# VITA-Group/Open-L2O

Measured on NVIDIA H100. Metric: coordinate-updates/sec (N_params x unroll_steps), higher is better.
Workload: dtype f32

## Files before the change

open_l2o_b200/csrc/cwlstm_tc.cuh:

```cuda
#pragma once
#include "cwlstm_common.cuh"
#include "l2o_internal.h"

namespace l2o {
namespace tc {

constexpr int kH = 20;
constexpr int kN = 4 * kH;
constexpr int kTile = 64;
constexpr int kU = 5;
constexpr int kFwdWG = 3;
constexpr int kFwdThreads = 128 * kFwdWG;
template <int N>
struct IC {
  static constexpr int value = N;
};

template <class C>
struct Geo {
  static constexpr bool FC = C::FC;
  static constexpr int ColH1 = FC ? 24 : 4, ColH2 = FC ? 44 : 24;
  static constexpr int ColOne = FC ? 20 : C::F;
  static constexpr int KB = FC ? 8 : 6;
  static constexpr int L1Lo = 0, L1Hi = FC ? 6 : 3;
  static constexpr int L2Lo = FC ? 2 : 0, L2Hi = KB;
  static constexpr int K1 = 8 * (L1Hi - L1Lo), K2 = 8 * (L2Hi - L2Lo);
  static constexpr int N1 = FC ? 48 : 24, N2 = 48;
  static constexpr int B1Floats = K1 * kN, B2Floats = K2 * kN, T1Floats = kN * N1, T2Floats = kN * N2;
  static constexpr int FwdFloats = 2 * (B1Floats + B2Floats);
  static constexpr int AllFloats = FwdFloats + 2 * (T1Floats + T2Floats);
  static_assert(!FC || C::F == 20, "fc preprocessing: dim 20");
  static_assert(FC || C::F <= 3, "feature chunk: at most 3 features");
};
constexpr int kImgMaxFloats = Geo<Cfg<L2O_PRE_FC, 2, 20, 20, 20>>::AllFloats;

__device__ __forceinline__ uint32_t smem_u32(const void* p) { return (uint32_t)__cvta_generic_to_shared(p); }

__device__ __forceinline__ void mbar_init(uint64_t* bar, uint32_t count) {
  asm volatile("mbarrier.init.shared::cta.b64 [%0], %1;" ::"r"(smem_u32(bar)), "r"(count));
}
__device__ __forceinline__ void mbar_expect_tx(uint64_t* bar, uint32_t bytes) {
  asm volatile("mbarrier.arrive.expect_tx.shared::cta.b64 _, [%0], %1;" ::"r"(smem_u32(bar)), "r"(bytes) : "memory");
}
__device__ __forceinline__ void mbar_wait(uint64_t* bar, uint32_t parity) {
  asm volatile(
      "{\n\t"
      ".reg .pred p;\n\t"
      "WAIT_LOOP:\n\t"
      "mbarrier.try_wait.parity.shared::cta.b64 p, [%0], %1;\n\t"
      "@p bra WAIT_DONE;\n\t"
      "bra WAIT_LOOP;\n\t"
      "WAIT_DONE:\n\t"
      "}\n" ::"r"(smem_u32(bar)),
      "r"(parity)
      : "memory");
}
__device__ __forceinline__ void fence_barrier_init() { asm volatile("fence.mbarrier_init.release.cluster;" ::: "memory"); }
__device__ __forceinline__ void fence_proxy_async() { asm volatile("fence.proxy.async.shared::cta;" ::: "memory"); }
__device__ __forceinline__ void tma_bulk_g2s(void* dst, const void* src, uint32_t bytes, uint64_t* bar) {
  asm volatile("cp.async.bulk.shared::cluster.global.mbarrier::complete_tx::bytes [%0], [%1], %2, [%3];" ::"r"(
                   smem_u32(dst)),
               "l"(src), "r"(bytes), "r"(smem_u32(bar))
               : "memory");
}
__device__ __forceinline__ void stage_image(float* dst, const float* src, uint32_t bytes, uint64_t* bar) {
  if (threadIdx.x == 0) {
    mbar_expect_tx(bar, bytes);
    tma_bulk_g2s(dst, src, bytes, bar);
  }
  mbar_wait(bar, 0);
}

__device__ __forceinline__ void wg_fence() { asm volatile("wgmma.fence.sync.aligned;" ::: "memory"); }
__device__ __forceinline__ void wg_commit() { asm volatile("wgmma.commit_group.sync.aligned;" ::: "memory"); }
template <int N>
__device__ __forceinline__ void wg_wait() {
  asm volatile("wgmma.wait_group.sync.aligned %0;" ::"n"(N) : "memory");
}

__device__ __forceinline__ uint64_t make_desc(uint32_t saddr, uint32_t lbo, uint32_t sbo) {
  return (uint64_t)((saddr & 0x3FFFFu) >> 4) | ((uint64_t)(lbo >> 4) << 16) | ((uint64_t)(sbo >> 4) << 32);
}
__device__ __forceinline__ uint64_t img_desc(const float* p, int ncols) {
  return make_desc(smem_u32(p), (uint32_t)(ncols / 8) * 128u, 128u);
}
__host__ __device__ constexpr uint64_t img_kstep(int ncols) { return (uint64_t)((2 * (ncols / 8) * 128) >> 4); }

#define L2O_ACC8(b) "+f"(d[b]), "+f"(d[b + 1]), "+f"(d[b + 2]), "+f"(d[b + 3]), "+f"(d[b + 4]), "+f"(d[b + 5]), \
                    "+f"(d[b + 6]), "+f"(d[b + 7])
__device__ __forceinline__ void mma_rs_n80(float* d, const uint32_t* a, uint64_t b, uint32_t acc) {
  asm volatile(
      "{\n\t.reg .pred p;\n\tsetp.ne.b32 p, %45, 0;\n\t"
      "wgmma.mma_async.sync.aligned.m64n80k8.f32.tf32.tf32 "
      "{%0,%1,%2,%3,%4,%5,%6,%7,%8,%9,%10,%11,%12,%13,%14,%15,%16,%17,%18,%19,"
      "%20,%21,%22,%23,%24,%25,%26,%27,%28,%29,%30,%31,%32,%33,%34,%35,%36,%37,%38,%39}, "
      "{%40,%41,%42,%43}, %44, p, 1, 1;\n\t}\n"
      : L2O_ACC8(0), L2O_ACC8(8), L2O_ACC8(16), L2O_ACC8(24), L2O_ACC8(32)
      : "r"(a[0]), "r"(a[1]), "r"(a[2]), "r"(a[3]), "l"(b), "r"(acc));
}
__device__ __forceinline__ void mma_rs_n48(float* d, const uint32_t* a, uint64_t b, uint32_t acc) {
  asm volatile(
      "{\n\t.reg .pred p;\n\tsetp.ne.b32 p, %29, 0;\n\t"
      "wgmma.mma_async.sync.aligned.m64n48k8.f32.tf32.tf32 "
      "{%0,%1,%2,%3,%4,%5,%6,%7,%8,%9,%10,%11,%12,%13,%14,%15,%16,%17,%18,%19,%20,%21,%22,%23}, "
      "{%24,%25,%26,%27}, %28, p, 1, 1;\n\t}\n"
      : L2O_ACC8(0), L2O_ACC8(8), L2O_ACC8(16)
      : "r"(a[0]), "r"(a[1]), "r"(a[2]), "r"(a[3]), "l"(b), "r"(acc));
}
__device__ __forceinline__ void mma_rs_n24(float* d, const uint32_t* a, uint64_t b, uint32_t acc) {
  asm volatile(
      "{\n\t.reg .pred p;\n\tsetp.ne.b32 p, %17, 0;\n\t"
      "wgmma.mma_async.sync.aligned.m64n24k8.f32.tf32.tf32 "
      "{%0,%1,%2,%3,%4,%5,%6,%7,%8,%9,%10,%11}, "
      "{%12,%13,%14,%15}, %16, p, 1, 1;\n\t}\n"
      : L2O_ACC8(0), "+f"(d[8]), "+f"(d[9]), "+f"(d[10]), "+f"(d[11])
      : "r"(a[0]), "r"(a[1]), "r"(a[2]), "r"(a[3]), "l"(b), "r"(acc));
}
template <int N>
__device__ __forceinline__ void mma_rs(float* d, const uint32_t* a, uint64_t b, uint32_t acc) {
  static_assert(N == 80 || N == 48 || N == 24, "wgmma width");
  if constexpr (N == 80) mma_rs_n80(d, a, b, acc);
  else if constexpr (N == 48) mma_rs_n48(d, a, b, acc);
  else mma_rs_n24(d, a, b, acc);
}

__device__ __forceinline__ float to_tf32(float x) {
  uint32_t r;
  asm("cvt.rna.tf32.f32 %0, %1;" : "=r"(r) : "f"(x));
  return __uint_as_float(r);
}
__device__ __forceinline__ void split_tf32(float x, uint32_t& hi, uint32_t& lo) {
  hi = __float_as_uint(x) & 0xFFFFE000u;
  lo = __float_as_uint(x - __uint_as_float(hi));
}

__host__ __device__ constexpr int vec_unit(int c, int base) { return 5 * ((c - base) & 3) + ((c - base) >> 2); }
__host__ __device__ constexpr int unit_col(int u, int base) { return base + 4 * (u % 5) + u / 5; }
__host__ __device__ constexpr int gate_ref_col(int n) {
  return (2 * ((n >> 3) & 1) + (n & 1)) * kH + 5 * ((n & 7) >> 1) + (n >> 4);
}
__host__ __device__ constexpr int dx_gate_col(int k) { return (k & ~7) + 2 * (k & 3) + ((k >> 2) & 1); }
__host__ __device__ constexpr int dx_group(int c) { return c / 24; }
__host__ __device__ constexpr int dx_unit(int c) {
  return 2 * ((c % 24) >> 3) + (c & 1) >= 5 ? -1 : 5 * ((c & 7) >> 1) + 2 * ((c % 24) >> 3) + (c & 1);
}
__host__ __device__ constexpr int img_index(int k, int n, int ncols) {
  return ((k >> 2) * (ncols / 8) + (n >> 3)) * 32 + (n & 7) * 4 + (k & 3);
}

template <class C>
__device__ __forceinline__ float ext_weight(const float* __restrict__ theta, bool l2, int c, int n) {
  using G = Geo<C>;
  const int col = gate_ref_col(n);
  if (c == G::ColOne) return theta[(l2 ? C::O_B2 : C::O_B1) + col];
  const bool in_h1 = c >= G::ColH1 && c < G::ColH1 + kH, in_h2 = c >= G::ColH2 && c < G::ColH2 + kH;
  if (!l2) {
    if (in_h1) return theta[C::O_W1 + (C::F + vec_unit(c, G::ColH1)) * C::G1 + col];
    if (G::FC && c < kH) return theta[C::O_W1 + vec_unit(c, 0) * C::G1 + col];
    if (!G::FC && c < C::F) return theta[C::O_W1 + c * C::G1 + col];
    return 0.f;
  }
  if (in_h1) return theta[C::O_W2 + vec_unit(c, G::ColH1) * C::G2 + col];
  if (in_h2) return theta[C::O_W2 + (kH + vec_unit(c, G::ColH2)) * C::G2 + col];
  return 0.f;
}
template <class C>
__host__ __device__ constexpr int dx_operand_col(bool l2, int c) {
  using G = Geo<C>;
  return l2 ? unit_col(dx_unit(c), dx_group(c) == 0 ? G::ColH1 : G::ColH2)
            : unit_col(dx_unit(c), dx_group(c) == 0 ? G::ColH1 : 0);
}

template <class C>
__global__ void prep_weights_kernel(const float* __restrict__ theta, float* __restrict__ img, int with_transposed) {
  static_assert(C::H1 == kH && C::H2 == kH && (C::F <= 3 || C::FC), "tc engine: LSTM-20x2, F <= 3 or fc(20)");
  using G = Geo<C>;
  const int nb = (G::K1 + G::K2) * kN;
  const int nt = with_transposed ? kN * (G::N1 + G::N2) : 0;
  for (int e = blockIdx.x * blockDim.x + threadIdx.x; e < nb + nt; e += gridDim.x * blockDim.x) {
    float w;
    float* hi;
    int off, idx;
    if (e < nb) {
      const bool l2 = e >= G::K1 * kN;
      const int ee = l2 ? e - G::K1 * kN : e;
      const int k = ee / kN, n = ee % kN;
      w = ext_weight<C>(theta, l2, 8 * (l2 ? G::L2Lo : G::L1Lo) + k, n);
      hi = img + (l2 ? 2 * G::B1Floats : 0);
      off = l2 ? G::B2Floats : G::B1Floats;
      idx = img_index(k, n, kN);
    } else {
      const int e2 = e - nb;
      const bool l2 = e2 >= kN * G::N1;
      const int nc = l2 ? G::N2 : G::N1;
      const int ee = l2 ? e2 - kN * G::N1 : e2;
      const int k = ee / nc, n = ee % nc;
      w = dx_unit(n) < 0 ? 0.f : ext_weight<C>(theta, l2, dx_operand_col<C>(l2, n), dx_gate_col(k));
      hi = img + G::FwdFloats + (l2 ? 2 * G::T1Floats : 0);
      off = l2 ? G::T2Floats : G::T1Floats;
      idx = img_index(k, n, nc);
    }
    const float h = to_tf32(w);
    hi[idx] = h;
    hi[off + idx] = to_tf32(w - h);
  }
}

template <int KB>
struct Frag {
  uint32_t hi[KB][4], lo[KB][4];
  __device__ __forceinline__ void zero() {
#pragma unroll
    for (int k = 0; k < KB; ++k)
#pragma unroll
      for (int r = 0; r < 4; ++r) { hi[k][r] = 0u; lo[k][r] = 0u; }
  }
  __device__ __forceinline__ void put_at(int c, int rh, float v) {
    split_tf32(v, hi[c / 8][((c / 4) & 1) * 2 + rh], lo[c / 8][((c / 4) & 1) * 2 + rh]);
  }
  __device__ __forceinline__ float get_at(int c, int rh) const {
    return __uint_as_float(hi[c / 8][((c / 4) & 1) * 2 + rh]) + __uint_as_float(lo[c / 8][((c / 4) & 1) * 2 + rh]);
  }
  template <int COL>
  __device__ __forceinline__ void put(int rh, float v) {
    static_assert(COL % 4 == 0 && COL / 8 < KB, "fragment column");
    put_at(COL, rh, v);
  }
  template <int BASE>
  __device__ __forceinline__ void put_vec(int rh, const float* v) {
    static_assert(BASE % 4 == 0 && (BASE + 19) / 8 < KB, "fragment column");
#pragma unroll
    for (int s = 0; s < kU; ++s) put_at(BASE + 4 * s, rh, v[s]);
  }
};

template <int N, int KB, int LO, int HI>
__device__ __forceinline__ void mma3(float* d, const Frag<KB>& f, uint64_t bh, uint64_t bl) {
  constexpr uint64_t step = img_kstep(N);
#pragma unroll
  for (int kb = LO; kb < HI; ++kb) {
    const uint64_t o = (uint64_t)(kb - LO) * step;
    mma_rs<N>(d, f.lo[kb], bh + o, kb > LO ? 1u : 0u);
    mma_rs<N>(d, f.hi[kb], bl + o, 1u);
    mma_rs<N>(d, f.hi[kb], bh + o, 1u);
  }
}

__host__ __device__ constexpr int acc_idx(int s, int g, int rh) { return 4 * (2 * s + (g >> 1)) + 2 * rh + (g & 1); }

constexpr float kLog2e = 1.4426950408889634f;
__device__ __forceinline__ void lstm_point_fwd(float zi, float zj, float zf, float zo, float& c, float& h) {
  const float Ei = ex2_approx(fminf(-kLog2e * zi, 40.f));
  const float Ej = ex2_approx(fminf(-2.f * kLog2e * zj, 40.f));
  const float Qf = 1.0f + ex2_approx(fminf(fmaf(-kLog2e, zf, -kLog2e), 40.f));
  const float Pij = (1.0f + Ei) * (1.0f + Ej);
  const float cn = fmaf(c, Pij, (1.0f - Ej) * Qf) * rcp_approx(Pij * Qf);
  c = cn;
  const float Ec = ex2_approx(fminf(-2.f * kLog2e * cn, 63.f));
  const float Eo = ex2_approx(fminf(-kLog2e * zo, 63.f));
  h = (1.0f - Ec) * rcp_approx((1.0f + Ec) * (1.0f + Eo));
}
__device__ __forceinline__ float elu_fast(float av) {
  const float em = ex2_approx(kLog2e * av) - 1.0f;
  const float ep = av * fmaf(av, fmaf(av, fmaf(av, 1.0f / 24.0f, 1.0f / 6.0f), 0.5f), 1.0f);
  return av > 0.f ? av : (av > -0.0625f ? ep : em);
}

__device__ __forceinline__ void load5(const float* __restrict__ p, int q, float* v) {
#pragma unroll
  for (int s = 0; s < kU; ++s) v[s] = p[5 * q + s];
}
__device__ __forceinline__ void store5(float* __restrict__ p, int q, const float* v) {
#pragma unroll
  for (int s = 0; s < kU; ++s) p[5 * q + s] = v[s];
}
__device__ __forceinline__ float quad_sum(float v) {
  v += __shfl_xor_sync(0xffffffffu, v, 1);
  return v + __shfl_xor_sync(0xffffffffu, v, 2);
}
__device__ __forceinline__ float from_row(float v, int lane, int rh) {
  return __shfl_sync(0xffffffffu, v, (lane & ~3) | rh);
}

struct FwdExtra {
  const int32_t* step_ptr;
  int32_t t_offset;
  float p_fixed;
};

template <class C>
struct SmemF {
  float img[Geo<C>::FwdFloats];
  float wo[kH + 4];
  float win[64];
  uint64_t wbar;
};
template <class C>
__host__ __device__ constexpr size_t adamc_offset() {
  return (sizeof(SmemF<C>) + 15) & ~(size_t)15;
}
template <class C>
__host__ __device__ constexpr size_t fwd_smem_bytes(int T) {
  return adamc_offset<C>() + (C::FC ? (size_t)T * 2 * sizeof(float) : 0);
}
__device__ __forceinline__ double warp_sum_pairs_d(double v) {
  v += __shfl_xor_sync(0xffffffffu, v, 16);
  v += __shfl_xor_sync(0xffffffffu, v, 8);
  v += __shfl_xor_sync(0xffffffffu, v, 4);
  return v + __shfl_xor_sync(0xffffffffu, v, 1);
}

template <class C, bool FAST = false, int OPT = L2O_OPT_NONE, bool CKPT = false>
__global__ void __launch_bounds__(kFwdThreads, 1) unroll_fwd_kernel(l2o_unroll_args a, NetRt rt, const float* __restrict__ img,
                                                                     float* __restrict__ state_out, FwdExtra ex) {
  static_assert(!FAST || (!C::FC && OPT != L2O_OPT_NONE), "the full-tile forward is the DM nets' with an optimizee");
  using G = Geo<C>;
  extern __shared__ __align__(128) unsigned char smem_raw[];
  SmemF<C>& S = *reinterpret_cast<SmemF<C>*>(smem_raw);
  const int T = a.T;
  const int64_t n = a.n;
  const bool in_kernel_opt = FAST || a.opt_kind != L2O_OPT_NONE;
  const int opt_kind = FAST ? OPT : a.opt_kind;
  const bool want_fx = in_kernel_opt && a.fx != nullptr;
  const bool adam_mode = C::NIN == 2 && a.m != nullptr;
  const bool has_ckpt = FAST ? CKPT : a.ckpt != nullptr;
  const bool has_grec = FAST ? CKPT : a.g_rec != nullptr;
  const bool tanh_out = !FAST && rt.tanh_output;
  const bool has_delta = !FAST && a.delta_seq != nullptr;
  const bool has_labels = !FAST && a.labels != nullptr;
  float* adamc = reinterpret_cast<float*>(smem_raw + adamc_offset<C>());

  if (threadIdx.x < kH) S.wo[threadIdx.x] = a.theta[C::O_WO + threadIdx.x];
  if (threadIdx.x == kH) S.wo[kH] = a.theta[C::O_BO];
  if constexpr (C::FC) {
    static_assert(!C::FC || C::NIN == 2, "fc nets here are RNNprop nets (two inputs)");
    if (threadIdx.x >= 32 && threadIdx.x < 92) S.win[threadIdx.x - 32] = a.theta[C::O_WIN + threadIdx.x - 32];
    if (adam_mode) {
      const int step0 = ex.step_ptr ? *ex.step_ptr + ex.t_offset : a.step0;
      for (int t = threadIdx.x; t < T; t += blockDim.x) {
        const float p = (ex.step_ptr == nullptr && ex.p_fixed > 0.f) ? ex.p_fixed : (float)(step0 + t);
        adamc[2 * t] = 1.0f - powf(a.beta1, p);
        adamc[2 * t + 1] = 1.0f - powf(a.beta2, p);
      }
    }
  }
  if (threadIdx.x == 0) {
    mbar_init(&S.wbar, 1);
    fence_barrier_init();
  }
  __syncthreads();
// ... 261 lines not shown
```

open_l2o_b200/csrc/cwlstm_tc_bwd.cuh:

```cuda
#pragma once
#include <type_traits>
#include "cwlstm_tc.cuh"

namespace l2o {
namespace tcb {

using namespace tc;

constexpr int kBwdWG = 2;
constexpr int kBwdThreads = 128 * kBwdWG;
constexpr uint32_t kXaLBO = 8 * 128;
constexpr uint32_t kXbLBO = 10 * 128;
constexpr uint32_t kXaBytes = 8 * kXaLBO;
constexpr uint32_t kXbBytes = 8 * kXbLBO;
constexpr int kBlkL1 = 5, kRowOne2 = 63;

__device__ __forceinline__ void split_bf16x2(float v0, float v1, uint32_t& hi, uint32_t& lo) {
  asm("cvt.rn.bf16x2.f32 %0, %1, %2;" : "=r"(hi) : "f"(v1), "f"(v0));
  const float r0 = v0 - __uint_as_float(hi << 16), r1 = v1 - __uint_as_float(hi & 0xFFFF0000u);
  asm("cvt.rn.bf16x2.f32 %0, %1, %2;" : "=r"(lo) : "f"(r1), "f"(r0));
}
__device__ __forceinline__ void stsm_x4_trans(uint32_t sa, uint32_t r0, uint32_t r1, uint32_t r2, uint32_t r3) {
  asm volatile("stmatrix.sync.aligned.m8n8.x4.trans.shared.b16 [%0], {%1, %2, %3, %4};" ::"r"(sa), "r"(r0), "r"(r1),
               "r"(r2), "r"(r3)
// ... 194 lines not shown
      split_bf16x2(z[4 * j + 2], z[4 * j + 3], h1, l1);
      stsm_x4_trans(lb + (uint32_t)j * 128, h0, h1, l0, l1);
    }
  };
  auto dx_dw = [&](auto ncols, float* z, float* x, uint64_t th, uint64_t tl, uint64_t xah, uint64_t xal) {
    constexpr int NX = decltype(ncols)::value;
    uint32_t fh[kN / 8][4], fl[kN / 8][4];
#pragma unroll
    for (int j = 0; j < kN / 8; ++j) {
      split_tf32(z[4 * j + 0], fh[j][0], fl[j][0]);
      split_tf32(z[4 * j + 2], fh[j][1], fl[j][1]);
      split_tf32(z[4 * j + 1], fh[j][2], fl[j][2]);
      split_tf32(z[4 * j + 3], fh[j][3], fl[j][3]);
    }
    constexpr uint64_t step = img_kstep(NX);
    wg_fence();
#pragma unroll
    for (int j = 0; j < kN / 8; ++j) {
      mma_rs<NX>(x, fl[j], th + j * step, j > 0 ? 1u : 0u);
      mma_rs<NX>(x, fh[j], tl + j * step, 1u);
      mma_rs<NX>(x, fh[j], th + j * step, 1u);
    }
    wg_commit();
    constexpr uint64_t sa = (2 * kXaLBO) >> 4, sb = (2 * kXbLBO) >> 4;
#pragma unroll
    for (int kk = 0; kk < tc::kTile / 16; ++kk) {
      mma_ss_bf16_n80(dw, xal + kk * sa, xbh + kk * sb);
      mma_ss_bf16_n80(dw, xah + kk * sa, xbl + kk * sb);
      mma_ss_bf16_n80(dw, xah + kk * sa, xbh + kk * sb);
    }
    wg_commit();
    wg_wait<1>();
  };
  auto flush_dw = [&]() {
    wg_wait<0>();
#pragma unroll
    for (int rh = 0; rh < 2; ++rh) {
      const int r = dw_row<C, MODE>(kx + 8 * rh);
#pragma unroll
      for (int j = 0; j < kN / 8; ++j)
#pragma unroll
        for (int e = 0; e < 2; ++e) {
          float& v = dw[4 * j + 2 * rh + e];
          if (r >= 0 && v != 0.f) atomicAdd(&a.dtheta[r + gate_ref_col(8 * j + 2 * q + e)], (double)v);
          v = 0.f;
        }
    }
  };

  for (int64_t tile = (int64_t)blockIdx.x * kBwdWG + wg; tile < ntiles; tile += tstride) {
    const int64_t r0 = tile * tc::kTile + kx;
    const int64_t row[2] = {r0, r0 + 8};
    const bool act[2] = {FULL || row[0] < n, FULL || row[1] < n};
    const float* ckt = a.ckpt + (int64_t)(T - 1) * slot + tile * tc::kTile * kH;
    int64_t tn = (int64_t)(T - 1) * n;
    float dc2[2][kU], dh2c[2][kU], dc1[2][kU], dh1c[2][kU];
#pragma unroll
    for (int rh = 0; rh < 2; ++rh)
#pragma unroll
      for (int s = 0; s < kU; ++s) { dc2[rh][s] = 0.f; dh2c[rh][s] = 0.f; dc1[rh][s] = 0.f; dh1c[rh][s] = 0.f; }
    float lam[2];
#pragma unroll
    for (int rh = 0; rh < 2; ++rh) lam[rh] = (kL2 && act[rh] && !kImit) ? a.g_rec[tn + n + row[rh]] : 0.f;
    if constexpr (CARRY) {
#pragma unroll
      for (int rh = 0; rh < 2; ++rh) {
        if (!act[rh]) continue;
        const int64_t i = row[rh];
        if constexpr (kL2) {
          load5(cy.d_state + (2 * n + i) * kH, q, dh2c[rh]);
          load5(cy.d_state + (3 * n + i) * kH, q, dc2[rh]);
          lam[rh] = cy.lam[i] + a.g_rec[tn + n + i];
        }
        if constexpr (kL1) {
          load5(cy.d_state + i * kH, q, dh1c[rh]);
          load5(cy.d_state + (n + i) * kH, q, dc1[rh]);
        }
      }
    }
    A.zero();
    A.template put<(G::ColOne & ~3)>(0, q == (G::ColOne & 3) ? 1.0f : 0.f);
    A.template put<(G::ColOne & ~3)>(1, q == (G::ColOne & 3) ? 1.0f : 0.f);

    for (int t = T - 1; t >= 0; --t) {
      const float* ckr = ckt + kx * kH;
      float z[kN / 2];
      float dh1n[2][kU];
      if constexpr (kL2) {
        float c2p[2][kU], dy[2];
        if constexpr (kRing) mbar_wait(&R.barh, 0);
#pragma unroll
        for (int rh = 0; rh < 2; ++rh) {
          float h1n[kU] = {0.f, 0.f, 0.f, 0.f, 0.f}, h2p[kU] = {0.f, 0.f, 0.f, 0.f, 0.f};
#pragma unroll
          for (int s = 0; s < kU; ++s) c2p[rh][s] = 0.f;
          float dtanh = 1.0f;
          if (act[rh]) {
            const float* cr = ckr + 8 * kH * rh;
            if constexpr (kRing) {
              if (t == T - 1) load5(cr + slot, q, h1n);
              ring5(R.h, rh, true, h2p);
            } else {
              load5(cr + slot, q, h1n);
              load5(cr + 2 * nkh, q, h2p);
              load5(cr + 3 * nkh, q, c2p[rh]);
            }
            if constexpr (kImit) lam[rh] = (a.delta_seq[tn + row[rh]] - a.labels[tn + row[rh]]) * inv_nt;
            if constexpr (kTanh) {
              const float th = a.delta_seq[tn + row[rh]] / rt.scale;
              dtanh = fmaf(-th, th, 1.0f);
            }
          }
          dy[rh] = rt.scale * lam[rh] * dtanh;
          if (!kRing || t == T - 1) A.template put_vec<G::ColH1>(rh, h1n);
          A.template put_vec<G::ColH2>(rh, h2p);
        }
        wg_fence();
        mma3<kN, G::KB, G::L2Lo, G::L2Hi>(z, A, b2h, b2l);
        wg_commit();
        wg_wait<0>();
        if constexpr (kRing) {
          mbar_wait(&R.bar2, ph);
#pragma unroll
          for (int rh = 0; rh < 2; ++rh) ring5(R.c2, rh, act[rh], c2p[rh]);
        }
        if (q == 0) acc_bo += dy[0] + dy[1];
#pragma unroll
        for (int rh = 0; rh < 2; ++rh)
#pragma unroll
          for (int s = 0; s < kU; ++s) {
            float hn;
            unit_bwd(z[acc_idx(s, 0, rh)], z[acc_idx(s, 1, rh)], z[acc_idx(s, 2, rh)], z[acc_idx(s, 3, rh)], c2p[rh][s],
                     fmaf(wo[s], dy[rh], dh2c[rh][s]), dc2[rh][s], hn);
            acc_wo[s] = fmaf(hn, dy[rh], acc_wo[s]);
          }
        wg_bar(wg);
        if constexpr (kRing) {
          if (elected) {
            const int64_t tl_next = t > 0 ? tile : tile + tstride;
            arm(&R.barh, R.h, ckt, 0, tile_bytes(tile));
            if (tl_next < ntiles) arm(&R.bar2, R.c2, t > 0 ? ckt - slot : ckt + ck_wrap, 3, tile_bytes(tl_next));
          }
        }
        stage_x(kXa2, 0, kBlkL1, G::ColH1, G::ColH2);
        stage_dz(z);
        fence_proxy_async();
        wg_bar(wg);
        float x2[G::N2 / 2];
        dx_dw(IC<G::N2>{}, z, x2, t2h, t2l, xa2h, xa2l);
#pragma unroll
        for (int rh = 0; rh < 2; ++rh)
#pragma unroll
          for (int s = 0; s < kU; ++s) {
            dh1n[rh][s] = x2[4 * (s >> 1) + 2 * rh + (s & 1)];
            dh2c[rh][s] = x2[4 * (3 + (s >> 1)) + 2 * rh + (s & 1)];
          }
        if constexpr (MODE == 1) {
#pragma unroll
          for (int rh = 0; rh < 2; ++rh)
            if (act[rh]) store5(a.scratch + (tn + row[rh]) * kH, q, dh1n[rh]);
        }
#pragma unroll
        for (int rh = 0; rh < 2; ++rh)
          if (!kImit && act[rh] && (!CARRY || t > 0)) lam[rh] += a.g_rec[tn + row[rh]];
      }
      if constexpr (kL1) {
        float c1p[2][kU];
        float r0v[2] = {0.f, 0.f};
        [[maybe_unused]] float r1v[2] = {0.f, 0.f};
        [[maybe_unused]] float ep[2][kU];
        if constexpr (kRing) mbar_wait(&R.barh, 1);
#pragma unroll
        for (int rh = 0; rh < 2; ++rh) {
          float h1p[kU] = {0.f, 0.f, 0.f, 0.f, 0.f};
#pragma unroll
          for (int s = 0; s < kU; ++s) c1p[rh][s] = 0.f;
          if (act[rh]) {
            if constexpr (kRing) {
              ring5(R.h, rh, true, h1p);
            } else {
              load5(ckr + 8 * kH * rh, q, h1p);
              load5(ckr + nkh + 8 * kH * rh, q, c1p[rh]);
            }
            if constexpr (MODE == 2) {
              load5(a.scratch + (tn + row[rh]) * kH, q, dh1n[rh]);
              r0v[rh] = a.in_seq[2 * tn + row[rh]];
              r1v[rh] = a.in_seq[2 * tn + n + row[rh]];
            } else {
              r0v[rh] = a.in_seq[tn + row[rh]];
            }
          } else if constexpr (MODE == 2) {
#pragma unroll
            for (int s = 0; s < kU; ++s) dh1n[rh][s] = 0.f;
          }
          A.template put_vec<G::ColH1>(rh, h1p);
          if constexpr (MODE == 2) {
            float e[kU];
#pragma unroll
            for (int s = 0; s < kU; ++s) {
              const int u = 5 * q + s;
              const float av = fmaf(r1v[rh], S.win[kH + u], fmaf(r0v[rh], S.win[u], S.win[2 * kH + u]));
              e[s] = elu_fast(av);
              ep[rh][s] = av > 0.f ? 1.0f : e[s] + 1.0f;
            }
            A.template put_vec<0>(rh, e);
          } else {
            float f[C::F];
            preprocess<C>(nullptr, rt, r0v[rh], 0.f, f);
            float v = q == C::F ? 1.0f : 0.f;
#pragma unroll
            for (int k = 0; k < C::F; ++k)
              if (q == k) v = f[k];
            A.template put<0>(rh, v);
          }
        }
        wg_fence();
        mma3<kN, G::KB, G::L1Lo, G::L1Hi>(z, A, b1h, b1l);
        wg_commit();
        wg_wait<0>();
        if constexpr (kRing) {
          mbar_wait(&R.bar1, ph);
#pragma unroll
          for (int rh = 0; rh < 2; ++rh) ring5(R.c1, rh, act[rh], c1p[rh]);
        }
#pragma unroll
        for (int rh = 0; rh < 2; ++rh)
#pragma unroll
          for (int s = 0; s < kU; ++s) {
            float hn;
            unit_bwd(z[acc_idx(s, 0, rh)], z[acc_idx(s, 1, rh)], z[acc_idx(s, 2, rh)], z[acc_idx(s, 3, rh)], c1p[rh][s],
                     dh1c[rh][s] + dh1n[rh][s], dc1[rh][s], hn);
          }
        wg_bar(wg);
        if constexpr (kRing) {
          const int64_t tl_next = t > 0 ? tile : tile + tstride;
          if (elected && tl_next < ntiles) {
            const float* ckn = t > 0 ? ckt - slot : ckt + ck_wrap;
            const uint32_t b = tile_bytes(tl_next);
            arm(&R.barh, R.h, ckn, 2, b);
            arm(&R.bar1, R.c1, ckn, 1, b);
            prefetch_l2_bulk(ck_block(ckn, 0), b);
          }
          const int64_t rn = t > 0 ? r0 : r0 + tstride * tc::kTile;
          const float* in_next = a.in_seq + (t > 0 ? tn - n : (int64_t)(T - 1) * n) + rn;
#pragma unroll
          for (int rh = 0; rh < 2; ++rh)
            if (q == 0 && ((FULL && t > 0) || rn + 8 * rh < n)) prefetch_l2(in_next + 8 * rh);
          ph ^= 1u;
        }
        if constexpr (MODE == 2) stage_x(kXa2, 0, kBlkL1, G::ColH1, 0);
        else stage_x(kXa1, kBlkL1, 3, G::ColH1, 0);
        stage_dz(z);
        fence_proxy_async();
        wg_bar(wg);
        float x1[G::N1 / 2];
        dx_dw(IC<G::N1>{}, z, x1, t1h, t1l, xa1h, xa1l);
#pragma unroll
        for (int rh = 0; rh < 2; ++rh)
#pragma unroll
          for (int s = 0; s < kU; ++s) {
            dh1c[rh][s] = x1[4 * (s >> 1) + 2 * rh + (s & 1)];
            if constexpr (MODE == 2) {
              const float da = x1[4 * (3 + (s >> 1)) + 2 * rh + (s & 1)] * ep[rh][s];
              aw0[s] = fmaf(r0v[rh], da, aw0[s]);
              aw1[s] = fmaf(r1v[rh], da, aw1[s]);
              ab[s] += da;
            }
          }
      }
      ckt -= slot;
      tn -= n;
    }
    if constexpr (CARRY) {
#pragma unroll
      for (int rh = 0; rh < 2; ++rh) {
        if (!act[rh]) continue;
        const int64_t i = row[rh];
        if constexpr (kL2) {
          store5(cy.d_state + (2 * n + i) * kH, q, dh2c[rh]);
          store5(cy.d_state + (3 * n + i) * kH, q, dc2[rh]);
          if (q == 0) cy.lam[i] = lam[rh];
        }
        if constexpr (kL1) {
          store5(cy.d_state + i * kH, q, dh1c[rh]);
          store5(cy.d_state + (n + i) * kH, q, dc1[rh]);
        }
      }
    }
    flush_dw();
  }
  wg_wait<0>();
  auto red8 = [&](float v) {
#pragma unroll
    for (int o = 4; o < 32; o <<= 1) v += __shfl_xor_sync(0xffffffffu, v, o);
    return v;
  };
#pragma unroll
  for (int s = 0; s < kU; ++s) {
    const int u = 5 * q + s;
    if constexpr (kL2) {
      const float v = red8(acc_wo[s]);
      if (lane < 4) atomicAdd(&a.dtheta[C::O_WO + u], (double)v);
    }
    if constexpr (MODE == 2) {
      const float v0 = red8(aw0[s]), v1 = red8(aw1[s]), vb = red8(ab[s]);
      if (lane < 4) {
        atomicAdd(&a.dtheta[C::O_WIN + u], (double)v0);
        atomicAdd(&a.dtheta[C::O_WIN + C::F + u], (double)v1);
        atomicAdd(&a.dtheta[C::O_BIN + u], (double)vb);
      }
    }
  }
  if constexpr (kL2) {
    const float v = red8(acc_bo);
    if (lane == 0) atomicAdd(&a.dtheta[C::O_BO], (double)v);
  }
}

}

template <class C, bool CARRY>
int tc_launch_bwd(const char* fn, const NetRt& rt, const l2o_bwd_args& a, float* img, cudaStream_t st, int sms,
                  const l2o_bwd_carry& cy) {
  tc::prep_weights_kernel<C><<<16, 256, 0, st>>>(a.theta, img, 1);
  if (int rc = after_launch(fn)) return rc;
  const int64_t ntiles = (a.n + tc::kTile - 1) / tc::kTile;
  const int64_t ctas = (ntiles + tcb::kBwdWG - 1) / tcb::kBwdWG;
  const int grid = (int)(ctas < sms ? ctas : sms);
  auto launch = [&](auto kern, size_t smem) {
    if (smem > 227 * 1024) return L2O_E_INVALID;
    if (int rc = raise_smem_limit(fn, kern, smem)) return rc;
    kern<<<grid, tcb::kBwdThreads, smem, st>>>(a, rt, img, cy);
    return after_launch(fn);
  };
  const int fl = (a.labels != nullptr ? tcb::kFlImit : 0) | (rt.tanh_output ? tcb::kFlTanh : 0);
  auto launch_l2 = [&](auto mode, auto full) {
    constexpr int M = decltype(mode)::value;
    constexpr bool F = decltype(full)::value;
    constexpr size_t smem = tcb::bwd_smem_bytes<C, M>();
    switch (fl) {
      case 0: return launch(tcb::unroll_bwd_kernel<C, M, CARRY, 0, F>, smem);
      case tcb::kFlImit: return launch(tcb::unroll_bwd_kernel<C, M, CARRY, tcb::kFlImit, F>, smem);
      case tcb::kFlTanh: return launch(tcb::unroll_bwd_kernel<C, M, CARRY, tcb::kFlTanh, F>, smem);
      default: return launch(tcb::unroll_bwd_kernel<C, M, CARRY, tcb::kFlImit | tcb::kFlTanh, F>, smem);
    }
  };
  if constexpr (C::FC) {
    int rc = launch_l2(tc::IC<1>{}, std::false_type{});
    if (rc != L2O_OK) return rc;
    return launch(tcb::unroll_bwd_kernel<C, 2, CARRY, 0, false>, tcb::bwd_smem_bytes<C, 2>());
  } else {
    if (a.n % tc::kTile == 0) return launch_l2(tc::IC<0>{}, std::true_type{});
    return launch_l2(tc::IC<0>{}, std::false_type{});
  }
}

}
```

open_l2o_b200/meta.py:

```python
from __future__ import annotations

import collections
import os

import numpy as np
import torch

from . import engine as _engine
from . import networks
from .variables import variable_getter

_PRODUCER_KINDS = ("lasso_batch", "mlp_xent", "confocal_psf")
MetaLoss = collections.namedtuple("MetaLoss", "loss, update, reset, fx, x")
MetaStep = collections.namedtuple("MetaStep", "step, update, reset, fx, x")


class Op(object):

    def __init__(self, kind, program):
        self.kind, self.program = kind, program

    def __repr__(self):
        return "<l2o op {}>".format(self.kind)

# ... 430 lines not shown
            h.step(r.net.theta, r.g_rec[t], r.ckpt[j * slot:(j + 1) * slot], r.ckpt[(j + 1) * slot:(j + 2) * slot],
                   reuse_weights=(j > 0), **kw)

    def _state_slot(self, r, t):
        slot = r.slot
        if not r.seg:
            return r.ckpt[t * slot:(t + 1) * slot]
        k = self._bound_index.get(t)
        if k is not None:
            return r.bstate[k]
        return r.ckpt[(t % 2) * slot:(t % 2 + 1) * slot]

    def _forward_external(self, train, step0):
        T, Xw = self.T, self._Xw
        self._fused_regime = False
        Xw.copy_(self.X)
        fxs = []
        for r in self.runs:
            self._state_slot(r, 0).copy_(r.state)
            self._load_moments(r)
        for t in range(T):
            fx, g = self._value_and_grad(Xw)
            fxs.append(fx)
            for r in self.runs:
                h = r.net.handle
                r.g_rec[t].copy_(g[r.off:r.off + r.n])
                kw = {}
                if h.n_in == 2:
                    if r.seg and t in self._bound_index:
                        r.bmv[self._bound_index[t], 0].copy_(r.m_work)
                        r.bmv[self._bound_index[t], 1].copy_(r.v_work)
                    kw = self._moments(r.m_work, r.v_work, step_ptr=self.step_dev, t_offset=t, feat_out=r.feat_rec[t])
                if train and r.delta_rec is not None:
                    kw["delta"] = r.delta_rec[t]
                h.step(r.net.theta, r.g_rec[t], self._state_slot(r, t), self._state_slot(r, t + 1),
                       x=Xw[r.off:r.off + r.n], reuse_weights=(t > 0), **kw)
        if train:
            fx, g = self._value_and_grad(Xw)
            for r in self.runs:
                r.g_rec[T].copy_(g[r.off:r.off + r.n])
        else:
            if self.producer is not None:
                fx = self._produce(Xw)[0]
            else:
                with torch.no_grad():
                    fx = self._loss_at(Xw)
        fxs.append(fx)
        for r in self.runs:
            r.state_final = self._state_slot(r, T)
        return torch.stack([f.reshape(()).double() for f in fxs])

    def _graph_body(self, train, step0):
        fx = self._forward_external(train, step0)
        if train:
            self._bptt()
        return fx

    def _bptt(self):
        for d in self.dtheta.values():
            d.zero_()
        for r in self.runs:
            h = r.net.handle
            in_seq = r.feat_rec if h.n_in == 2 else r.g_rec
            if not r.seg:
                h.unroll_bwd(r.net.theta, r.n, self.T, in_seq, r.ckpt, self.dtheta[r.key], g_rec=r.g_rec,
                             **self._bwd_extra(r))
                continue
            r.d_state.zero_()
            r.lam.zero_()
            for k in reversed(range(len(self.plan.bounds) - 1)):
                t0, t1 = self.plan.bounds[k], self.plan.bounds[k + 1]
                self._recompute(r, k)
                kw = {} if r.delta_rec is None else {"delta_seq": r.delta_rec[t0:]}
                h.unroll_bwd_carry(r.net.theta, r.n, t1 - t0, in_seq[t0:], r.ckpt, self.dtheta[r.key], r.d_state, r.lam,
                                   g_rec=r.g_rec[t0:], scratch=r.bwd_scratch, **kw)

    @staticmethod
    def _bwd_extra(r):
        kw = {}
        if r.delta_rec is not None:
            kw["delta_seq"] = r.delta_rec
        if r.bwd_scratch is not None:
            kw["scratch"] = r.bwd_scratch
        return kw

    def _graph_eligible(self):
        return os.environ.get("L2O_CUDA_GRAPH", "1") != "0" and self.fused is None and not self.scale_active

    def _run_external(self, train, step0):
        self.step_dev.fill_(int(step0))
        key = bool(train)
        if not self._graph_eligible() or self._graph_failed:
            return self._graph_body(train, step0)
        self._eager_calls[key] = self._eager_calls.get(key, 0) + 1
        if self._eager_calls[key] <= 2:
            return self._graph_body(train, step0)
        if key not in self._graphs:
            try:
                import gc
                gc.collect()
                torch.cuda.synchronize()
                g = torch.cuda.CUDAGraph()
                n0 = _engine.launch_count()
                with torch.cuda.graph(g):
                    fx = self._graph_body(train, step0)
                self._graph_kernels[key] = _engine.launch_count() - n0
                self._graphs[key] = (g, fx, [r.state_final for r in self.runs])
            except Exception as e:
                import warnings
                warnings.warn("CUDA-graph capture of the unroll failed (%r); staying eager" % (e,))
                self._graph_failed = True
                torch.cuda.synchronize()
                return self._graph_body(train, step0)
        g, fx, finals = self._graphs[key]
        g.replay()
        _engine.note_graph_replay(self._graph_kernels[key])
        for r, f in zip(self.runs, finals):
            r.state_final = f
        return fx

    def execute(self, kinds, feed):
        if kinds == {"reset"}:
            self.reset()
            return {}
        if "reset" in kinds:
            raise ValueError("fetch `reset` on its own (the reference runs it separately, DM/util.py:37)")
        out, mt = {}, collections.defaultdict(set)
        for k in kinds:
            if ":" in k:
                kind, ti = k.split(":")
                mt[int(ti)].add(kind)
        for ti in sorted(mt):
            out.update(self.mt_tasks[ti].execute(mt[ti], feed))
        kinds = set(k for k in kinds if ":" not in k)
        if mt and not kinds:
            return out
        train = "step" in kinds
        step0 = self._step0(feed)
        self._apply_scale_feed(feed)
        if self.fused is not None and not self.scale_active:
            fx = self._forward_fused(train, step0)
            if train:
                self._bptt()
        else:
            fx = self._run_external(train, step0)
        if train:
            if self.opt.distributed:
                from .dist import allreduce_meta_grad
                fx = allreduce_meta_grad(self.dtheta, fx)
        elif self.opt.distributed:
            import torch.distributed as dist
            fx = fx.clone()
            dist.all_reduce(fx)
        if "loss" in kinds:
            out["loss"] = float(fx.sum().item())
        if "fx" in kinds:
            out["fx"] = float(fx[self.T].item())
        if "x" in kinds:
            out["x"] = self.x_values(self._Xw)
        self.last_fx = fx
        if train:
            _adam_step(self.nets, self.dtheta, self.adam, self.learning_rate)
            out["step"] = None
        if "update" in kinds:
            self.X.copy_(self._Xw)
            for r in self.runs:
                r.state.copy_(r.state_final)
                if r.net.handle.n_in == 2:
                    r.m.copy_(r.m_work)
                    r.v.copy_(r.v_work)
            self.unroll_idx += 1
            out["update"] = None
        return out


class _MtTask(object):

    def __init__(self, prog, index):
        self.prog, self.index = prog, index
        T = prog.T
        self.subsets = []
        for key, subset in zip(prog.net_keys, prog.subsets):
            runs = [r for r in prog.runs if r.key == key]
            if len(runs) != 1:
                raise NotImplementedError("imitation tasks need each net's variables contiguous in the arena")
            r = runs[0]
            h = r.net.handle
            if getattr(r.net, "per_variable", False):
                raise NotImplementedError("imitation tasks are implemented for the coordinate-wise nets")
            sb = dict(run=r, n=r.n, state=h.new_state(r.n, prog.device),
                      ckpt=torch.zeros((T + 1) * r.slot, device=prog.device),
                      dseq=torch.zeros(T * r.n, device=prog.device),
                      inp=Placeholder("mt{}_input_subset{}".format(index, len(self.subsets))),
                      lab=Placeholder("mt{}_label_subset{}".format(index, len(self.subsets))))
            if h.n_in == 2:
                sb.update(m=torch.zeros(r.n, device=prog.device), v=torch.zeros(r.n, device=prog.device),
                          feat=torch.zeros(T, 2, r.n, device=prog.device))
            if r.bwd_scratch is not None and prog.segmented:
                sb["scratch"] = torch.zeros(T, r.n, 20, device=prog.device)
            self.subsets.append(sb)
        self.n_total = sum(sb["n"] for sb in self.subsets)
        self.adam = _adam_slots(prog.nets)
        self.il = torch.zeros(1, dtype=torch.float64, device=prog.device)

    def _dev(self, arr, T, n):
        t = torch.as_tensor(np.asarray(arr, dtype=np.float32)) if not torch.is_tensor(arr) else arr.float()
        return t.reshape(T, n).to(self.prog.device).contiguous()

    def execute(self, kinds, feed):
        prog, T = self.prog, self.prog.T
        if kinds == {"reset_mt"}:
            for sb in self.subsets:
                sb["state"].zero_()
                if "m" in sb:
                    sb["m"].zero_()
                    sb["v"].zero_()
            return {}
        train, commit = "step_mt" in kinds, "update_mt" in kinds
        self.il.zero_()
        if train:
            for d in prog.dtheta.values():
                d.zero_()
        finals = []
        step0 = prog._step0(feed)
        for sb in self.subsets:
            r, n = sb["run"], sb["n"]
            h = r.net.handle
            inp, lab = self._dev(feed[sb["inp"]], T, n), self._dev(feed[sb["lab"]], T, n)
            work, moments, kw, in_seq = sb["state"].clone(), None, {}, inp
            if h.n_in == 2:
                moments = (sb["m"].clone(), sb["v"].clone())
                kw, in_seq = prog._moments(*moments, step0=step0, feat_rec=sb["feat"]), sb["feat"]
            h.unroll_fwd(r.net.theta, n, T, work, in_seq=inp, ckpt=sb["ckpt"] if train else None, labels=lab,
                         imit_loss=self.il, n_total=self.n_total, delta_seq=sb["dseq"] if train else None, **kw)
            if train:
                extra = dict(prog._bwd_extra(r), delta_seq=sb["dseq"])
                if "scratch" in sb:
                    extra["scratch"] = sb["scratch"]
                h.unroll_bwd(r.net.theta, n, T, in_seq, sb["ckpt"], prog.dtheta[r.key], labels=lab, n_total=self.n_total,
                             **extra)
            finals.append((work, moments))
        out = {}
        if "loss_mt" in kinds:
            out["loss_mt:%d" % self.index] = float(self.il.item())
        if train:
            _adam_step(prog.nets, prog.dtheta, self.adam, prog.learning_rate)
            out["step_mt:%d" % self.index] = None
        if commit:
            for sb, (w, moments) in zip(self.subsets, finals):
                sb["state"].copy_(w)
                if moments is not None:
                    sb["m"].copy_(moments[0])
                    sb["v"].copy_(moments[1])
            out["update_mt:%d" % self.index] = None
        return out


class MetaOptimizer(object):

    beta1 = 0.95
    beta2 = 0.95

    def __init__(self, **kwargs):
        self._nets = None
        self.seed = int(kwargs.pop("_seed", 0))
        self.distributed = bool(kwargs.pop("_distributed", False))
        self.bptt_segment = kwargs.pop("_bptt_segment", None)
        if not kwargs:
            self._config = {
                "coordinatewise": {
                    "net": "CoordinateWiseDeepLSTM",
                    "net_options": {
                        "layers": (20, 20),
                        "preprocess_name": "LogAndSign",
                        "preprocess_options": {"k": 5},
                        "scale": 0.01,
                    }}}
        else:
            self._config = kwargs

    def save(self, sess=None, path=None, index=None):
        result = {}
        for k, net in self._nets.items():
            if path is None:
                filename, key = None, k
            elif index is not None:
                filename = os.path.join(path, "{}.l2l-{}".format(k, index))
                key = filename
            else:
                filename = os.path.join(path, "{}.l2l".format(k))
                key = filename
            result[key] = networks.save(net, sess, filename=filename)
        return result

    def restore(self, sess, path, index):
        for k, net in self._nets.items():
            with open(os.path.join(path, "{}.l2l-{}".format(k, index)), "rb") as f:
                data = networks._pickle.load(f)
            for m, v, shp in net.variable_shapes():
                if m not in data or v not in data[m] or tuple(np.shape(data[m][v])) != tuple(shp):
                    raise ValueError("{}.l2l-{}: variable {}/{} missing or of the wrong shape".format(k, index, m, v))
            net.set_variables(data)

    def meta_loss(self, make_loss, len_unroll, net_assignments=None, second_derivatives=False):
        prog = _Program(self, make_loss, len_unroll, net_assignments, second_derivatives)
        self.program = prog
        self.step_placeholder = prog.step_placeholder
        return MetaLoss(Op("loss", prog), Op("update", prog), Op("reset", prog), Op("fx", prog), Op("x", prog))

    def meta_minimize(self, make_loss, len_unroll, learning_rate=0.01, **kwargs):
        info = self.meta_loss(make_loss, len_unroll, **kwargs)
        self.program.learning_rate = learning_rate
        return MetaStep(Op("step", self.program), *info[1:])


class RNNpropMetaOptimizer(MetaOptimizer):

    def __init__(self, beta1=0.95, beta2=0.95, **kwargs):
        super(RNNpropMetaOptimizer, self).__init__(**kwargs)
        self.beta1, self.beta2 = beta1, beta2
```

Before: 1.922 billion.

## Narrow backward transposed wgmma to n40 and skip state copy in fused path

Packs the backward dx operand columns more densely, so the transposed weight images use 40 columns instead of 48 and the backward uses m64n40 wgmma instead of n48. New dx_slot/dx_reg helpers remap unit-to-register indexing to match. Separately, meta.py swaps the state tensor reference instead of copying it when running fused without CUDA graphs, and moves the host .item() syncs after the update copies. Together these cut tensor-core work, device copies and the point where the host stalls; the aliasing of state and state_final carries a risk if either buffer is reused later.

Measured after the change: 1.948 billion (median of 6 runs). 1.3% higher.

```diff
diff --git a/open_l2o_b200/csrc/cwlstm_tc.cuh b/open_l2o_b200/csrc/cwlstm_tc.cuh
--- a/open_l2o_b200/csrc/cwlstm_tc.cuh
+++ b/open_l2o_b200/csrc/cwlstm_tc.cuh
@@ -25,7 +25,7 @@
   static constexpr int L1Lo = 0, L1Hi = FC ? 6 : 3;
   static constexpr int L2Lo = FC ? 2 : 0, L2Hi = KB;
   static constexpr int K1 = 8 * (L1Hi - L1Lo), K2 = 8 * (L2Hi - L2Lo);
-  static constexpr int N1 = FC ? 48 : 24, N2 = 48;
+  static constexpr int N1 = FC ? 40 : 24, N2 = 40;
   static constexpr int B1Floats = K1 * kN, B2Floats = K2 * kN, T1Floats = kN * N1, T2Floats = kN * N2;
   static constexpr int FwdFloats = 2 * (B1Floats + B2Floats);
   static constexpr int AllFloats = FwdFloats + 2 * (T1Floats + T2Floats);
@@ -98,13 +98,13 @@
       : L2O_ACC8(0), L2O_ACC8(8), L2O_ACC8(16), L2O_ACC8(24), L2O_ACC8(32)
       : "r"(a[0]), "r"(a[1]), "r"(a[2]), "r"(a[3]), "l"(b), "r"(acc));
 }
-__device__ __forceinline__ void mma_rs_n48(float* d, const uint32_t* a, uint64_t b, uint32_t acc) {
+__device__ __forceinline__ void mma_rs_n40(float* d, const uint32_t* a, uint64_t b, uint32_t acc) {
   asm volatile(
-      "{\n\t.reg .pred p;\n\tsetp.ne.b32 p, %29, 0;\n\t"
-      "wgmma.mma_async.sync.aligned.m64n48k8.f32.tf32.tf32 "
-      "{%0,%1,%2,%3,%4,%5,%6,%7,%8,%9,%10,%11,%12,%13,%14,%15,%16,%17,%18,%19,%20,%21,%22,%23}, "
-      "{%24,%25,%26,%27}, %28, p, 1, 1;\n\t}\n"
-      : L2O_ACC8(0), L2O_ACC8(8), L2O_ACC8(16)
+      "{\n\t.reg .pred p;\n\tsetp.ne.b32 p, %25, 0;\n\t"
+      "wgmma.mma_async.sync.aligned.m64n40k8.f32.tf32.tf32 "
+      "{%0,%1,%2,%3,%4,%5,%6,%7,%8,%9,%10,%11,%12,%13,%14,%15,%16,%17,%18,%19}, "
+      "{%20,%21,%22,%23}, %24, p, 1, 1;\n\t}\n"
+      : L2O_ACC8(0), L2O_ACC8(8), "+f"(d[16]), "+f"(d[17]), "+f"(d[18]), "+f"(d[19])
       : "r"(a[0]), "r"(a[1]), "r"(a[2]), "r"(a[3]), "l"(b), "r"(acc));
 }
 __device__ __forceinline__ void mma_rs_n24(float* d, const uint32_t* a, uint64_t b, uint32_t acc) {
@@ -118,10 +118,10 @@
 }
 template <int N>
 __device__ __forceinline__ void mma_rs(float* d, const uint32_t* a, uint64_t b, uint32_t acc) {
-  static_assert(N == 80 || N == 48 || N == 24, "wgmma width");
+  static_assert(N == 80 || N == 40 || N == 24, "wgmma width");
   if constexpr (N == 80) mma_rs_n80(d, a, b, acc);
-  else if constexpr (N == 48) mma_rs_n48(d, a, b, acc);
-  else mma_rs_n24(d, a, b, acc);
+  else if constexpr (N == 40) mma_rs_n40(d, a, b, acc);
+  else if constexpr (N == 24) mma_rs_n24(d, a, b, acc);
 }
 
 __device__ __forceinline__ float to_tf32(float x) {
@@ -140,10 +140,12 @@
   return (2 * ((n >> 3) & 1) + (n & 1)) * kH + 5 * ((n & 7) >> 1) + (n >> 4);
 }
 __host__ __device__ constexpr int dx_gate_col(int k) { return (k & ~7) + 2 * (k & 3) + ((k >> 2) & 1); }
-__host__ __device__ constexpr int dx_group(int c) { return c / 24; }
-__host__ __device__ constexpr int dx_unit(int c) {
-  return 2 * ((c % 24) >> 3) + (c & 1) >= 5 ? -1 : 5 * ((c & 7) >> 1) + 2 * ((c % 24) >> 3) + (c & 1);
-}
+__host__ __device__ constexpr int dx_slot(int c) { return 2 * (c >> 3) + (c & 1); }
+__host__ __device__ constexpr int dx_group(int c) { return dx_slot(c) / kU; }
+__host__ __device__ constexpr int dx_unit(int c, int nc) {
+  return dx_slot(c) >= (nc == 40 ? 2 * kU : kU) ? -1 : 5 * ((c & 7) >> 1) + dx_slot(c) % kU;
+}
+__host__ __device__ constexpr int dx_reg(int i, int rh) { return 4 * (i >> 1) + 2 * rh + (i & 1); }
 __host__ __device__ constexpr int img_index(int k, int n, int ncols) {
   return ((k >> 2) * (ncols / 8) + (n >> 3)) * 32 + (n & 7) * 4 + (k & 3);
 }
@@ -167,8 +169,8 @@
 template <class C>
 __host__ __device__ constexpr int dx_operand_col(bool l2, int c) {
   using G = Geo<C>;
-  return l2 ? unit_col(dx_unit(c), dx_group(c) == 0 ? G::ColH1 : G::ColH2)
-            : unit_col(dx_unit(c), dx_group(c) == 0 ? G::ColH1 : 0);
+  return l2 ? unit_col(dx_unit(c, G::N2), dx_group(c) == 0 ? G::ColH1 : G::ColH2)
+            : unit_col(dx_unit(c, G::N1), dx_group(c) == 0 ? G::ColH1 : 0);
 }
 
 template <class C>
@@ -195,7 +197,7 @@
       const int nc = l2 ? G::N2 : G::N1;
       const int ee = l2 ? e2 - kN * G::N1 : e2;
       const int k = ee / nc, n = ee % nc;
-      w = dx_unit(n) < 0 ? 0.f : ext_weight<C>(theta, l2, dx_operand_col<C>(l2, n), dx_gate_col(k));
+      w = dx_unit(n, nc) < 0 ? 0.f : ext_weight<C>(theta, l2, dx_operand_col<C>(l2, n), dx_gate_col(k));
       hi = img + G::FwdFloats + (l2 ? 2 * G::T1Floats : 0);
       off = l2 ? G::T2Floats : G::T1Floats;
       idx = img_index(k, n, nc);
diff --git a/open_l2o_b200/csrc/cwlstm_tc_bwd.cuh b/open_l2o_b200/csrc/cwlstm_tc_bwd.cuh
--- a/open_l2o_b200/csrc/cwlstm_tc_bwd.cuh
+++ b/open_l2o_b200/csrc/cwlstm_tc_bwd.cuh
@@ -370,8 +370,8 @@
         for (int rh = 0; rh < 2; ++rh)
 #pragma unroll
           for (int s = 0; s < kU; ++s) {
-            dh1n[rh][s] = x2[4 * (s >> 1) + 2 * rh + (s & 1)];
-            dh2c[rh][s] = x2[4 * (3 + (s >> 1)) + 2 * rh + (s & 1)];
+            dh1n[rh][s] = x2[dx_reg(s, rh)];
+            dh2c[rh][s] = x2[dx_reg(kU + s, rh)];
           }
         if constexpr (MODE == 1) {
 #pragma unroll
@@ -477,9 +477,9 @@
         for (int rh = 0; rh < 2; ++rh)
 #pragma unroll
           for (int s = 0; s < kU; ++s) {
-            dh1c[rh][s] = x1[4 * (s >> 1) + 2 * rh + (s & 1)];
+            dh1c[rh][s] = x1[dx_reg(s, rh)];
             if constexpr (MODE == 2) {
-              const float da = x1[4 * (3 + (s >> 1)) + 2 * rh + (s & 1)] * ep[rh][s];
+              const float da = x1[dx_reg(kU + s, rh)] * ep[rh][s];
               aw0[s] = fmaf(r0v[rh], da, aw0[s]);
               aw1[s] = fmaf(r1v[rh], da, aw1[s]);
               ab[s] += da;
diff --git a/open_l2o_b200/meta.py b/open_l2o_b200/meta.py
--- a/open_l2o_b200/meta.py
+++ b/open_l2o_b200/meta.py
@@ -606,10 +606,6 @@
             import torch.distributed as dist
             fx = fx.clone()
             dist.all_reduce(fx)
-        if "loss" in kinds:
-            out["loss"] = float(fx.sum().item())
-        if "fx" in kinds:
-            out["fx"] = float(fx[self.T].item())
         if "x" in kinds:
             out["x"] = self.x_values(self._Xw)
         self.last_fx = fx
@@ -619,12 +615,19 @@
         if "update" in kinds:
             self.X.copy_(self._Xw)
             for r in self.runs:
-                r.state.copy_(r.state_final)
+                if self._fused_regime and not self._graphs:
+                    r.state = r.state_final
+                else:
+                    r.state.copy_(r.state_final)
                 if r.net.handle.n_in == 2:
                     r.m.copy_(r.m_work)
                     r.v.copy_(r.v_work)
             self.unroll_idx += 1
             out["update"] = None
+        if "loss" in kinds:
+            out["loss"] = float(fx.sum().item())
+        if "fx" in kinds:
+            out["fx"] = float(fx[self.T].item())
         return out
 
 
```
